# DaehwanKimLab/centrifuge

Measured on AMD Instinct MI355X. Metric: classified reads/sec (whole node) on 100bp synthetic reads vs p_compressed; HBM GB/s achieved, higher is better.
Workload: dtype u64

## Files before the change

### centrifuge_amd/csrc/cf_device.hip

```cpp
#include <hip/hip_runtime.h>
#include <sched.h>
#include <dlfcn.h>

#include <algorithm>
#include <cmath>
#include <chrono>
#include <cstdio>
#include <cstdlib>
#include <cstring>
#include <memory>
#include <mutex>
#include <stdexcept>
#include <string>
#include <vector>

#include "../../include/centrifuge_amd.h"
#include "cf_index.hpp"
#include "cf_kernels.hpp"
#include "cf_scan.hpp"
#include "cf_textio.hpp"
#include "cf_inflate.hpp"
#include "cf_restore.hpp"
#include "cf_plan.hpp"
#include "cf_knobs.hpp"
// ... 1285 lines not shown
    bt->maxLenHost = maxLen;
    const uint64_t nq = bt->nQueries;
    bt->bases.ensure(nWords + 16); bt->nmask.ensure(nWords + 16);
    bt->rlen.ensure(nReads + 16); bt->seeds.ensure(nReads + 1); bt->woff.ensure(nReads + 1);
    bt->pass.ensure(nReads + 1); bt->hitCap.ensure(nReads + 16);
    bt->slotOf.ensure(nReads + 1); bt->hitBase.ensure(nReads + 1); bt->items.ensure(nReads + 1);
    bt->nhml.ensure(2 * nReads + 1);
    bt->maxScore.ensure(nq + 1); bt->qflag.ensure(nq + 1); bt->qhead.ensure(nq + 1); bt->qRows.ensure(nq + 16); bt->qBase.ensure(nq + 1);
    bt->qplan.ensure((nq + 1) * kInlinePlan); bt->o1tax.ensure((nq + 1) * kFieldRows); bt->o1a.ensure((nq + 1) * kFieldRows); bt->o1b.ensure((nq + 1) * kFieldRows);
    bt->slowPost.ensure(nq + 1); bt->slowScore.ensure(nq + 1);
    if (envInt("CF_EARLY_SCORE", 0)) bt->postDeferred.ensure(nq + 16);
    bt->out.ensure(nq * (uint64_t)cl->d.k + 1); bt->nOut.ensure(nq + 16); bt->score2.ensure(nq + 1); bt->rowFirst.ensure(nq + 1);
    bt->cursor.ensure(4); bt->ops.ensure(1); bt->st.ensure(1);
    bt->tileA.ensure(scan_tiles_for(std::max(nReads, nq)) + 1); bt->tileC.ensure(scan_tiles_for(std::max(nReads, nq)) + 1);
    bt->recWords = searchVersion() != 2 ? 0u : maxLen <= 128 ? 4u : maxLen <= 192 ? 6u : maxLen <= 256 ? 8u : 0u;
    if ((uint64_t)(0.15 * maxLen) + maxLen / (uint64_t)ftc + 3 >= 255) bt->recWords = 0;
    bt->selfRecords = bt->recWords && cl->ix->d.planes && nWords < 0xffffffffull && envInt("CF_SELF_RECORDS", 1);
    if (bt->selfRecords) bt->itemMeta.ensure(8 * nReads + 8);
    bt->revDelta = bt->selfRecords && 2 * nWords + 64 < 0xffffffffull && envInt("CF_REV_WORDS", 1) ? (uint32_t)nWords + 16u : 0u;
    if (bt->revDelta) bt->bases.ensure(2 * (nWords + 16));
    else if (bt->recWords) bt->recs.ensure(2 * nReads * (uint64_t)rec_bytes((int)bt->recWords) + 64);
    uint64_t hitsWant = 2 * ((nBases ? nBases : 32 * nWords) / ftc + 2 * nReads);
    hitsWant += hitsWant / 50 + 4096;
    if (bt->hitsCapLimit) hitsWant = std::min(hitsWant, bt->hitsCapLimit);
    if (bt->hits.n < hitsWant) bt->hits.ensure(hitsWant);
    if (bt->recWords && bt->hits.n > 0xffffffffull) throw ArgError("batch too large: its hit lists need 32-bit offsets, split it");
    uint64_t rowsWant = std::max<uint64_t>(4 * nq, 1u << 16);
    if (bt->plannedPerQuery > 0) rowsWant = std::max<uint64_t>(rowsWant, (uint64_t)((double)nq * bt->plannedPerQuery * 1.15));
    if (const int per = envInt("CF_ROWS_PER_QUERY", 0)) rowsWant = std::max<uint64_t>((uint64_t)per * nq, 1024);
    if (bt->rowsCapLimit) rowsWant = bt->rowsCapLimit;
    if (bt->rowVal.n < rowsWant || bt->rowsCapLimit) { bt->rowVal.ensure(rowsWant); bt->rowRef.ensure(rowsWant); bt->hm.ensure(rowsWant); bt->tc.ensure(rowsWant); }
    bt->outCompact.ensure(nq * (uint64_t)cl->d.k + 1);
    bt->hSt.ensure(1); bt->hOps.ensure(1);
    bt->hNOut.ensure(nq + 1); bt->hScore2.ensure(nq + 1); bt->hMaxScore.ensure(nq + 1);
    if (bt->resultFormat == CF_RESULTS_NARROW) { bt->qinfo.ensure(nq + 16); bt->hQInfo.ensure(nq + 16); }
    bt->rowsSpec = bt->rowsPerQuery > 0 ? (uint64_t)((double)nq * bt->rowsPerQuery * 1.04) + 4096 : nq + nq / 4 + 1024;
    bt->rowsSpec = std::min<uint64_t>(bt->rowsSpec, nq * (uint64_t)cl->d.k);
    bt->hRows.ensure(std::max<uint64_t>(bt->rowsSpec, nq + nq / 4 + 1024));
    if (g_dryBytes) return;
    if (!bt->evInit) { for (auto &e : bt->ev) HIP_OK(hipEventCreate(&e)); HIP_OK(hipEventCreate(&bt->evLate)); HIP_OK(hipEventCreate(&bt->evPostFast)); HIP_OK(hipEventCreate(&bt->evPost)); bt->evInit = true; }
    if (!bt->tail && (envInt("CF_TAIL_STREAM", 0) || envInt("CF_EARLY_SCORE", 0))) HIP_OK(hipStreamCreateWithFlags(&bt->tail, hipStreamNonBlocking));
}

static void bindBatch(cf_batch *bt) {
    cf_classifier *cl = bt->cl;
    DPlan &pl = bt->pl;
    pl.nmask = bt->nmask.p; pl.rlen = bt->rlen.p; pl.woff = bt->woff.p; pl.nReads = (uint32_t)bt->nReads; pl.ftabChars = cl->ix->h.g.ftabChars;
    pl.maxLenAllowed = bt->maxLenHost;
    pl.nWords = bt->nWords;
    pl.pass = bt->pass.p; pl.hitCap = bt->hitCap.p; pl.slotOf = bt->slotOf.p;
    pl.hitBase = bt->hitBase.p; pl.items = bt->items.p; pl.st = bt->st.p;
    pl.itemMeta = bt->selfRecords ? bt->itemMeta.p : nullptr;
    pl.bases = bt->bases.p; pl.revDelta = bt->revDelta;
    pl.hitsCap = bt->hitsCapLimit ? std::min<uint64_t>(bt->hitsCapLimit, bt->hits.n) : bt->hits.n;
    DBatch &d = bt->d;
    d.bases = bt->bases.p; d.nmask = bt->nmask.p; d.rlen = bt->rlen.p; d.woff = bt->woff.p; d.seeds = bt->seeds.p;
    d.pass = bt->pass.p; d.items = bt->items.p; d.slotOf = bt->slotOf.p; d.hitBase = bt->hitBase.p; d.hitCap = bt->hitCap.p;
    d.lazyHits = (uint32_t)(envInt("CF_LAZY_HITS", 1) != 0) | (cl->ix->d.posFrag ? 4u : 0u);
    d.directRefs = (uint32_t)(cl->ix->dense.p && cl->ix->d.walkRate == 0 && envInt("CF_SCORE_FAST", 1) != 0 && envInt("CF_DIRECT_REFS", 1) != 0);
    d.hits = bt->hits.p; d.nhml = bt->nhml.p; d.qflag = bt->qflag.p; d.qhead = bt->qhead.p; d.qplan = bt->qplan.p; d.qplanStride = bt->qplan.n / kInlinePlan; d.qRows = bt->qRows.p; d.qBase = bt->qBase.p;
    d.rowVal = bt->rowVal.p; d.rowRef = bt->rowRef.p; d.hm = bt->hm.p; d.tc = bt->tc.p;
    d.out = bt->out.p; d.nOut = bt->nOut.p; d.score2 = bt->score2.p;
    d.counts = cl->counts.p; d.nTaxa = (uint32_t)cl->ix->h.taxa.size();
    d.nReads = (uint32_t)bt->nReads; d.nQueries = (uint32_t)bt->nQueries; d.paired = bt->paired;
    d.cursor = bt->cursor.p; d.st = bt->st.p; d.ops = bt->ops.p;
    d.slowPost = bt->slowPost.p; d.slowScore = bt->slowScore.p; d.postDeferred = envInt("CF_EARLY_SCORE", 0) ? bt->postDeferred.p : nullptr;
    d.o1tax = bt->o1tax.p; d.o1a = bt->o1a.p; d.o1b = bt->o1b.p; d.oStride = bt->o1tax.n / kFieldRows;
    d.hitsCap = pl.hitsCap;
    d.rowsCap = bt->rowsCapLimit ? std::min<uint64_t>(bt->rowsCapLimit, bt->rowVal.n) : bt->rowVal.n;
    d.recs = bt->recWords && !bt->selfRecords ? bt->recs.p : nullptr; d.recWords = bt->recWords;
    d.itemMeta = bt->selfRecords ? bt->itemMeta.p : nullptr;
}

static void enqueuePlan(cf_batch *bt, hipStream_t st) {
    const uint64_t nReads = bt->nReads;
    const DPlan &pl = bt->pl;
    HIP_OK(hipStreamWaitEvent(st, bt->ev[8], 0));
    if (bt->densePending) {
        const uint32_t L = bt->densePending - 1;
        const DUnpack u{bt->dense.p, bt->bases.p, bt->rlen.p, (uint32_t)nReads, L, bt->revDelta ? bt->bases.p + bt->revDelta : nullptr};
        bt->revMade = bt->revDelta != 0;
        const uint64_t threads = nReads * std::max<uint64_t>(((uint64_t)L + 31) >> 5, 1);
        hipLaunchKernelGGL(k_dense_unpack, dim3((unsigned)((threads + 255) / 256)), dim3(256), 0, st, u);
        bt->densePending = 0;
    }
    HIP_OK(hipEventRecord(bt->ev[5], st));
    HIP_OK(hipMemsetAsync(bt->st.p, 0, sizeof(BatchStatus), st));
    const dim3 gp((unsigned)((nReads + 1 + 255) / 256)), bl(256);
    if (bt->fromBytes && nReads) hipLaunchKernelGGL(k_rlen, gp, bl, 0, st, bt->off8.p, bt->rlen.p, (uint32_t)nReads);
    scan_enqueue<SCAN_WORDS>(bt->rlen.p, nReads, bt->woff.p, nullptr, bt->tileA.p, bt->tileC.p, st);
    if (bt->fromBytes && nReads) {
        DConvert c{bt->seq.p, bt->off8.p, bt->woff.p, bt->bases.p, bt->nmask.p, (uint32_t)nReads};
        hipLaunchKernelGGL(k_convert, dim3((unsigned)((nReads + 255) / 256)), dim3(256), 0, st, c);
    }
    if (bt->fromText && nReads) {
        const DTextPack c{bt->text.p, bt->txSeqOff.p, bt->rlen.p, bt->woff.p, bt->bases.p, bt->nmask.p, (uint32_t)nReads};
        hipLaunchKernelGGL(k_text_pack, dim3((unsigned)((nReads + 255) / 256)), dim3(256), 0, st, c);
    }
    hipLaunchKernelGGL(k_plan, gp, bl, 0, st, pl);
    scan_enqueue<SCAN_HITS>(bt->hitCap.p, nReads, bt->hitBase.p, bt->slotOf.p, bt->tileA.p, bt->tileC.p, st);
    hipLaunchKernelGGL(k_plan_fill, gp, bl, 0, st, pl);
    if (pl.revDelta && nReads && !bt->revMade) {
        const uint64_t threads = nReads * (uint64_t)bt->recWords;
        hipLaunchKernelGGL(k_rev_words, dim3((unsigned)((threads + 255) / 256)), bl, 0, st, pl, bt->recWords);
    }
    if (bt->nQueries) hipLaunchKernelGGL(k_plan_maxscore, dim3((unsigned)((bt->nQueries + 255) / 256)), bl, 0, st, bt->rlen.p, bt->pass.p,
// ... 1252 lines not shown
```

### centrifuge_amd/csrc/cf_kernels.hpp

```cpp
#pragma once
#include "cf_platform.hpp"

namespace cfamd {

constexpr uint32_t kNone32 = 0xffffffffu;
constexpr uint64_t kNone64 = ~0ull;
constexpr uint32_t kSideChars = 384;
constexpr int kSearchChunk = CF_WAVE;

struct RefInfo { uint64_t tax; uint32_t tidx, pid; };
static_assert(sizeof(RefInfo) == 16, "RefInfo layout");
struct DIndex {
    const uint8_t *sides;
    const uint64_t *ftab, *eftab;
    uint64_t fchr0, fchr1, fchr2, fchr3;
    uint64_t len, zOff, zSide;
    uint32_t zIn;
    int32_t ftabChars, offRate, offw;
    const void *offs;
    const uint8_t *planes;
    const uint8_t *planes2;
    const uint64_t *wide;
    int32_t wideChars;
    const uint64_t *text;
// ... 466 lines not shown
    uint64_t *rev;
};
CF_DEV void dense_unpack_body(const DUnpack &u, uint64_t t) {
    const uint32_t W = (u.readLen + 31) >> 5, bpr = (u.readLen + 3) >> 2;
    if (W == 0) { if (t < u.nReads) u.rlen[t] = 0; return; }
    const uint64_t r = t / W;
    const uint32_t k = (uint32_t)(t - r * W);
    if (r >= u.nReads) return;
    uint64_t w = load8_any(u.dense, r * bpr + 8ull * k);
    const uint32_t have = u.readLen - 32 * k;
    if (have < 32) w &= (1ull << (2 * have)) - 1;
    u.bases[r * W + k] = w;
    if (k == 0) u.rlen[r] = u.readLen;
    if (u.rev) {
        const uint32_t L = u.readLen;
        const int32_t s0 = (int32_t)(L - 1 - 32u * k) - 31;
        uint64_t x;
        if (s0 >= 0) {
            const uint64_t at = r * bpr + ((uint32_t)s0 >> 2);
            const uint32_t sh = 2u * ((uint32_t)s0 & 3u);
            x = load8_any(u.dense, at) >> sh;
            if (sh) x |= (load8_any(u.dense, at + 8) & 0xffull) << (64 - sh);
        } else x = load8_any(u.dense, r * bpr) << (2 * (uint32_t)(-s0));
        uint64_t rv = pair_reverse(x);
        if (have < 32) rv &= (1ull << (2 * have)) - 1;
        u.rev[r * W + k] = rv;
    }
}

CF_DEV void rlen_body(const uint64_t *off, uint32_t *rlen, uint32_t nReads, uint32_t r) {
    if (r >= nReads) return;
    const uint64_t l = off[r + 1] - off[r];
    rlen[r] = l > 0xffffffffull ? 0xffffffffu : (uint32_t)l;
}

struct DPlan {
    const uint32_t *nmask;
    const uint32_t *rlen;
    const uint64_t *woff;
    uint32_t nReads;
    int32_t ftabChars;
    uint32_t maxLenAllowed;
    uint64_t nWords;
    uint8_t *pass;
    uint32_t *hitCap;
    uint32_t *slotOf;
    uint64_t *hitBase;
    uint32_t *items;
    uint32_t *itemMeta;
    uint64_t *bases;
    uint32_t revDelta;
    BatchStatus *st;
    uint64_t hitsCap;
};

CF_DEV void plan_body(const DPlan &p, uint32_t r) {
    if (r < p.nReads) {
        const uint64_t L = p.rlen[r], wo = p.woff[r];
        uint32_t nN = 0;
        const bool inside = wo + ((L + 31) >> 5) <= p.nWords;
        if (!inside) cf_atomic_or(&p.st->flags, kStWordsOverflow);
        for (uint64_t k = 0; inside && 32 * k < L; k++) {
            uint32_t m = p.nmask[wo + k];
            if (L - 32 * k < 32) m &= (1u << (L - 32 * k)) - 1u;
            nN += (uint32_t)cf_popc32(m);
        }
        const uint64_t maxns = (uint64_t)(0.0 + (double)0.15f * (double)L);
        bool ok = inside && L >= 2 && nN <= maxns;
        if (ok && L > p.maxLenAllowed) { cf_atomic_or(&p.st->flags, kStLenOverflow); ok = false; }
        const uint32_t cap = ok ? (uint32_t)(nN + (L - nN) / (uint64_t)p.ftabChars + 2) : 0u;
        p.pass[r] = ok ? 1 : 0;
        p.hitCap[r] = cap;
    }
}

CF_DEV uint64_t rev_word(const uint64_t *rw, uint32_t L, uint32_t k) {
    const uint32_t have = L - 32u * k;
    const int32_t s0 = (int32_t)(L - 1 - 32u * k) - 31;
    uint64_t x;
    if (s0 >= 0) {
        const uint32_t wi = (uint32_t)s0 >> 5, sh = (uint32_t)s0 & 31;
        x = rw[wi] >> (2 * sh);
        if (sh) x |= rw[wi + 1] << (64 - 2 * sh);
    } else x = rw[0] << (2 * (uint32_t)(-s0));
    uint64_t w = pair_reverse(x);
    if (have < 32) w &= (1ull << (2 * have)) - 1;
    return w;
}

constexpr uint32_t kItemHasN = 0x80000000u;
constexpr uint32_t kItemPre = 0x40000000u;
CF_DEV void plan_fill_body(const DPlan &p, uint32_t r) {
    if (r > p.nReads) return;
    if (r == p.nReads) {
        const uint64_t need = p.hitBase[r];
        p.st->hitsNeed = need;
        if (need > p.hitsCap) { cf_atomic_or(&p.st->flags, kStHitsOverflow); p.st->nItems = 0; }
        else p.st->nItems = 2u * p.slotOf[r];
        return;
    }
    const uint32_t slot = p.slotOf[r];
    if (p.pass[r]) {
        p.items[slot] = r;
        if (p.itemMeta) {
            const uint32_t wo = (uint32_t)p.woff[r], L = p.rlen[r], hb = (uint32_t)p.hitBase[r];
            uint32_t any = 0;
            for (uint32_t k = 0; 32 * k < L; k++) {
                uint32_t mk = p.nmask[p.woff[r] + k];
                if (L - 32 * k < 32) mk &= (1u << (L - 32 * k)) - 1u;
                any |= mk;
            }
            const bool pre = p.revDelta && !any;
            const uint32_t Lf = L | (any ? kItemHasN : 0u) | (pre ? kItemPre : 0u);
            uint32_t *m = p.itemMeta + 8 * (size_t)slot;
            m[0] = pre ? wo + p.revDelta : wo; m[1] = Lf; m[2] = hb; m[3] = r;
            m[4] = wo; m[5] = Lf; m[6] = hb + p.hitCap[r]; m[7] = r;
        }
    } else p.slotOf[r] = kNone32;
}

CF_DEV void rev_words_body(const DPlan &p, uint32_t wordsPerRead, uint64_t t) {
    const uint64_t r = t / wordsPerRead;
    const uint32_t k = (uint32_t)(t - r * wordsPerRead);
    if (r >= p.nReads || !p.revDelta || !p.pass[r]) return;
    const uint32_t L = p.rlen[r];
    if (32u * k >= L) return;
    const uint64_t wo = p.woff[r];
    p.bases[wo + p.revDelta + k] = rev_word(p.bases + wo, L, k);
}

constexpr uint32_t kMaxScoreNever = 0xffffffffu;
CF_DEV void plan_maxscore_body(const uint32_t *rlen, const uint8_t *pass, uint32_t nQueries, int paired, uint32_t *maxScore, uint32_t q) {
    if (q >= nQueries) return;
    const uint32_t r0 = paired ? 2 * q : q;
    const uint64_t L0 = rlen[r0];
    const uint64_t s0 = L0 > 15 ? (L0 - 15) * (L0 - 15) : 0u;
    const bool p0 = pass[r0] != 0;
    uint64_t v = p0 ? s0 : 0u;
    if (paired) {
        const uint64_t L1 = rlen[r0 + 1];
        const uint64_t s1 = L1 > 15 ? (L1 - 15) * (L1 - 15) : 0u;
        const bool p1 = pass[r0 + 1] != 0;
        v = (p0 && p1) ? s0 + s1 : p0 ? s0 : p1 ? s1 : 0u;
    }
    maxScore[q] = v >= 0xffffffffull ? kMaxScoreNever : (uint32_t)v;
}

struct DCompact {
    const OutRow *out;
    const uint64_t *o1tax, *o1a, *o1b;
    uint64_t oStride;
    const uint32_t *nOut;
    const uint64_t *rowFirst;
    uint32_t k, nQueries;
    OutRow *dst;
    BatchStatus *st;
    NarrowRow *dstNarrow;
    uint8_t *qinfo;
    const uint8_t *pass;
    int32_t paired;
};
CF_DEV OutRow row_of_one(uint64_t tax, uint64_t a, uint64_t bb) {
    OutRow o; o.taxID = tax; o.uniqueID = (uint32_t)a; o.score = (uint32_t)(a >> 32); o.hitLen = (uint32_t)bb; o.tidx = (uint32_t)(bb >> 32);
    return o;
}
CF_DEV void compact_body(const DCompact &c, uint32_t q) {
    if (q == c.nQueries && c.st) c.st->rowsOut = c.rowFirst[q];
    if (q >= c.nQueries) return;
    const uint32_t n = c.nOut[q] < c.k ? c.nOut[q] : c.k;
// ... 411 lines not shown
                rank_any<1>(ix, c0, t1, b1, t2, b2, two);
                if (b2 > t2) m4 |= 1u << c0;
            }
            if (!m4) masked = false;
            mask |= m4 << (4 * c1);
        }
    }
    table[t] = wide_entry(top, bot - top, j - ftc, cap, masked, mask);
}

enum : int { S_IDLE = 0, S_REC = 1, S_CALL = 2, S_FTAB = 3, S_EXT = 4, S_EXTB = 5, S_FTABW = 6, S_POS = 7, S_TXT = 8, S_ISA = 9, S_REC2 = 10 };

constexpr uint32_t kLazyHits = 2;
constexpr uint32_t lazy_hits(int G, int W) { return G == 1 && W >= 6 ? 1u : kLazyHits; }
constexpr uint32_t kVerifyMinLeft = 12;

template <int G, int W, bool COUNT, bool BLOCKS = false, int LZN = 0, bool MULTI = false>
CF_DEV void search2_body(const DIndex &ix, const DParams &pr, const DBatch &b, uint8_t *ldsBlock) {
    static_assert(!BLOCKS || G == 1, "the planes are read one chain per lane");
    constexpr int PER = 8 / G;
    constexpr int RB = rec_bytes(W);
    constexpr int RCH = RB / (16 * G);
    constexpr int NV = BLOCKS ? (RCH > 2 ? RCH : 2) : PER;
    static_assert(RCH >= 1 && RCH <= NV, "record does not fit the load slot");
    constexpr uint32_t kRawPieces = W / 2 + (W + 3) / 4;
    static_assert(G != 1 || (int)kRawPieces <= NV, "packed read does not fit the load slot");
    struct Slot { u64x2 v[NV]; };
    const int sub = Grp<G>::sub();
    const uint32_t lane = cf_lane();
    const uint32_t leaderLane = lane & ~(uint32_t)(G - 1);
    constexpr int RBL = rec_lds_stride(W);
    uint8_t *lrec = ldsBlock + (size_t)(cf_local_thread() / G) * RBL;
    constexpr uint32_t LZ = LZN ? (uint32_t)LZN : lazy_hits(G, W);
    uint64_t *lhit = reinterpret_cast<uint64_t *>(ldsBlock + (size_t)(cf_block_threads() / G) * RBL +
                                                  (BLOCKS ? (size_t)0 : (size_t)cf_block_threads() * 4 * RankTab<G>::WORDS)) +
                     (size_t)(cf_local_thread() / G) * 2 * LZ;
    uint32_t *scr = BLOCKS ? nullptr : reinterpret_cast<uint32_t *>(ldsBlock + (size_t)(cf_block_threads() / G) * RBL) + (size_t)cf_local_thread() * RankTab<G>::WORDS;
    const uint64_t *lw = reinterpret_cast<const uint64_t *>(lrec);
    const uint32_t *lm = reinterpret_cast<const uint32_t *>(lrec + 8 * W);
    uint32_t *lmeta = reinterpret_cast<uint32_t *>(lrec + RB - 16);
    const uint32_t ftc = (uint32_t)ix.ftabChars;
    int mode = S_IDLE;
    uint32_t cur = 0, dep = 0;
    uint32_t nhmx = 0;
    uint64_t top = 0, bot = 0;
    uint64_t aux = 0;
    uint32_t vf = 0;
    uint32_t endDep = 0;
    uint32_t mv = 0;
    uint32_t lz = 0;
    uint32_t wnext = 0, wend = 0;
    bool exhausted = false;
    constexpr bool SELF = G == 1;
    u64x2 cmeta{0, 0};
    uint32_t cbase = 0, pend = 0;
    unsigned long long cFtab = 0, cPair = 0, cPair2 = 0, cSingle = 0, cFtabW = 0, cVerify = 0, cText = 0, cPos = 0;
    const int32_t posRate = ix.posRate;
    const int32_t isaRate = MULTI ? posRate : ix.isaRate;
    const uint32_t nItems = b.st->nItems;
    const uint32_t wideChars = (uint32_t)ix.wideChars;

    for (;;) {
        uint32_t item = 0;
        const bool selfRec = SELF && b.itemMeta != nullptr;
        auto takeMeta = [&](bool mine, uint32_t it) {
            const int src = (int)((mine ? it - cbase : lane) & (uint32_t)(CF_WAVE - 1));
            const uint32_t m0 = cf_shfl((uint32_t)cmeta.x, src), m1 = cf_shfl((uint32_t)(cmeta.x >> 32), src), m2 = cf_shfl((uint32_t)cmeta.y, src);
            if (mine) {
                aux = (uint64_t)m0 | ((uint64_t)(m1 & (kItemHasN | kItemPre)) << 32);
                lmeta[0] = m1 & ~(kItemHasN | kItemPre); lmeta[1] = m2; lmeta[2] = it;
                cf_compiler_fence();
                mode = S_REC2;
            }
        };
        if (selfRec && cf_ballot(mode == S_REC)) takeMeta(mode == S_REC, pend);
        const uint64_t idleMask = cf_ballot(mode == S_IDLE && sub == 0);
        if (idleMask) {
            bool fresh = false;
            if (wnext >= wend && !exhausted) {
                uint32_t base = 0;
                if (lane == 0) base = (uint32_t)cf_atomic_add(&b.cursor[0], (unsigned long long)kSearchChunk);
                base = cf_first_lane_u32(base);
                if (base >= nItems) { exhausted = true; wnext = wend = 0; }
                else {
                    wnext = base; wend = base + kSearchChunk < nItems ? base + kSearchChunk : nItems;
                    if (selfRec) {
                        cbase = base; fresh = true;
                        cmeta = base + lane < nItems ? cf_load16(reinterpret_cast<const uint8_t *>(b.itemMeta + 4 * (size_t)(base + lane))) : u64x2{0, 0};
                    }
                }
            }
            const uint32_t avail = wend - wnext;
            const uint32_t nIdle = (uint32_t)cf_popc64(idleMask);
            bool took = false;
            if (mode == S_IDLE) {
                const uint32_t rnk = (uint32_t)cf_popc64(idleMask & ((1ull << leaderLane) - 1));
                if (rnk < avail) { item = wnext + rnk; mode = S_REC; pend = item; took = true; }
            }
            wnext += nIdle < avail ? nIdle : avail;
            if (selfRec && !fresh && cf_ballot(took)) takeMeta(took, item);
        }
        if (cf_ballot(mode != S_IDLE) == 0) {
            if (exhausted) break;
            continue;
        }
        const bool anyN = cf_ballot((mode != S_IDLE && (lz & 2u) != 0) || (mode == S_REC2 && (aux >> 63) != 0) || (mode == S_REC && !selfRec)) != 0;
        auto iter = [&](auto lmx) __attribute__((always_inline)) {
        Slot sa;
        sa.v[0] = u64x2{0, 0};
        uint64_t sS = 0;
        uint32_t oT = 0, oB = 0;
        bool same = true, stepN = false;
        int c = 0;
        const uint8_t *ldp = nullptr;
        uint32_t nch = 0, strd = 16;
        if (posRate >= 0 && mode == S_EXT && !(vf & 25u) && bot - top == 1 && (vf >> 8) >= ix.verifyMinRun &&
            (top & ((1ull << posRate) - 1)) == 0 && lmeta[0] - dep >= kVerifyMinLeft) {
            mode = S_POS;
            if (COUNT) cVerify++;
        } else if (MULTI && G == 1 && posRate == 0 && ix.multiRows && mode == S_EXT && !(vf & 25u) && bot - top >= 2 && bot - top <= ix.multiRows &&
                   (vf >> 8) >= ix.multiMinRun && lmeta[0] - dep >= kVerifyMinLeft) {
            mv = 0x80000000u | ((uint32_t)(bot - top) << 20);
            endDep = dep;
            mode = S_POS;
            if (COUNT) cVerify++;
        }
        if (mode == S_POS) {
            const uint64_t row = top + ((MULTI && (mv >> 31)) ? (mv & 15u) : 0u);
            if (COUNT && (MULTI && (mv >> 31)) && (mv & 15u)) cText++;
            ldp = reinterpret_cast<const uint8_t *>(ix.saPos + 2 * ((row >> posRate) / 3)); nch = 1;
        } else if (mode == S_ISA) {
            ldp = reinterpret_cast<const uint8_t *>(ix.isa + 2 * ((aux >> isaRate) / 3)); nch = 1;
        } else if (mode == S_TXT) {
            if constexpr (G == 1) {
                const uint64_t b0 = aux >= 64 ? ((aux - 1) >> 5) - 1 : 0;
                ldp = reinterpret_cast<const uint8_t *>(ix.text) + 8 * b0; nch = 1;
            } else {
                const uint64_t b0 = aux >= 64 ? (aux - 64) >> 5 : 0;
                ldp = reinterpret_cast<const uint8_t *>(ix.text) + 8 * b0 + (size_t)sub * (32 / G); nch = 2 / G;
            }
            if (COUNT) cText++;
        } else if (mode == S_REC) {
            if (G == 1 && b.itemMeta) nch = 0;
            else { ldp = b.recs + (uint64_t)item * RB + (size_t)sub * (RB / G); nch = RCH; }
        } else if (G == 1 && mode == S_REC2) {
            ldp = reinterpret_cast<const uint8_t *>(b.bases + (uint32_t)aux); nch = (aux >> 63) ? kRawPieces : W / 2;
        } else if (mode == S_FTAB) {
            ldp = reinterpret_cast<const uint8_t *>(ix.ftab + aux); nch = 1;
        } else if (mode == S_FTABW) {
            ldp = reinterpret_cast<const uint8_t *>(ix.wide + aux); nch = 1;
        } else if (mode == S_EXT || mode == S_EXTB) {
            c = (int)((lw[dep >> 5] >> (2 * (dep & 31))) & 3);
            stepN = mode == S_EXT && ((lmx[dep >> 5] >> (dep & 31)) & 1u) != 0;
            if (!stepN) {
                if constexpr (BLOCKS) {
                    const uint64_t row = mode == S_EXT ? top : bot;
                    sS = row >> 6;
                    if (mode == S_EXT) {
                        oT = (uint32_t)row & 63u;
                        const uint64_t spread = bot - top;
                        same = (uint64_t)oT + spread <= 64;
                        oB = same ? oT + (uint32_t)spread : 0u;
                        const uint32_t d1 = dep + 1;
                        const bool pair = ix.planes2 && !(vf & 8u) && d1 < lmeta[0] && ((lmx[d1 >> 5] >> (d1 & 31)) & 1u) == 0 &&
                                          !((vf & 16u) && d1 >= endDep);
                        vf = pair ? (vf | 4u) : (vf & ~4u);
                    } else oB = (uint32_t)row & 63u;
                    if (vf & 4u) {
                        const uint32_t d1 = dep + 1;
                        const int c0 = (int)((lw[d1 >> 5] >> (2 * (d1 & 31))) & 3);
                        ldp = ix.planes2 + sS * 256 + 16 * (4 * c + c0); nch = 1;
                    } else { ldp = ix.planes + sS * 64 + 16 * c; nch = 1; }
                } else {
                    if (mode == S_EXT) {
                        sS = side_of(ix, top);
                        oT = (uint32_t)(top - sS * kSideChars);
                        const uint64_t spread = bot - top;
                        same = (uint64_t)oT + spread <= kSideChars;
                        oB = same ? oT + (uint32_t)spread : 0u;
                    } else {
                        sS = side_of(ix, bot);
                        oB = (uint32_t)(bot - sS * kSideChars);
                    }
                    ldp = ix.sides + sS * 128 + 16 * sub; nch = PER; strd = 16 * G;
                }
            }
        }
        if (nch) sa.v[0] = cf_load16(ldp);
        if (nch > 1) {
#pragma unroll
            for (int i = 1; i < NV; i++) {
                if ((uint32_t)i >= nch) continue;
                if (G == 1 && mode == S_REC2 && i >= W / 2) sa.v[i] = cf_load16(reinterpret_cast<const uint8_t *>(b.nmask + (uint32_t)aux) + 16 * (i - W / 2));
                else sa.v[i] = cf_load16(ldp + (size_t)i * strd);
            }
        }
        cf_wait_vmem();
        const u64x2 ft = sa.v[0];
// ... 108 lines not shown
                for (int k = 0; k < W; k++) {
                    const uint64_t v = (k & 1) ? sa.v[k / 2].y : sa.v[k / 2].x;
                    uint64_t w = 0;
                    if (32u * (uint32_t)k < L) {
                        const uint32_t have = L - 32u * (uint32_t)k;
                        w = fwd ? v : ~v;
                        if (have < 32) w &= (1ull << (2 * have)) - 1;
                    }
                    rw[k] = w; rm[k] = 0u;
                }
            } else {
#pragma unroll
            for (int i = 0; i < W / 2; i++) { rw[2 * i] = sa.v[i].x; rw[2 * i + 1] = sa.v[i].y; }
#pragma unroll
            for (int i = 0; i < (W + 3) / 4; i++) {
                const bool hasN = (aux >> 63) != 0;
                const uint64_t a = hasN ? sa.v[W / 2 + i].x : 0ull, bq = hasN ? sa.v[W / 2 + i].y : 0ull;
                if (4 * i + 0 < W) rm[4 * i + 0] = (uint32_t)a;
                if (4 * i + 1 < W) rm[4 * i + 1] = (uint32_t)(a >> 32);
                if (4 * i + 2 < W) rm[4 * i + 2] = (uint32_t)bq;
                if (4 * i + 3 < W) rm[4 * i + 3] = (uint32_t)(bq >> 32);
            }
            cf_compiler_fence();
            uint64_t fw_[W]; uint32_t fm_[W];
#pragma unroll
            for (int k = 0; k < W; k++) {
                uint64_t w = 0; uint32_t m = 0;
                if (32u * (uint32_t)k < L) {
                    const uint32_t have = L - 32u * (uint32_t)k;
                    if (fwd) {
                        const int32_t s0 = (int32_t)(L - 1 - 32u * (uint32_t)k) - 31;
                        uint64_t x; uint32_t mm;
                        if (s0 >= 0) {
                            const uint32_t wi = (uint32_t)s0 >> 5, sh = (uint32_t)s0 & 31;
                            x = lw[wi] >> (2 * sh); mm = lmx[wi] >> sh;
                            if (sh) { x |= lw[wi + 1] << (64 - 2 * sh); mm |= lmx[wi + 1] << (32 - sh); }
                        } else {
                            const uint32_t neg = (uint32_t)(-s0);
                            x = lw[0] << (2 * neg); mm = lmx[0] << neg;
                        }
                        w = pair_reverse(x); m = cf_brev32(mm);
                    } else { w = ~lw[k]; m = lmx[k]; }
                    if (have < 32) { w &= (1ull << (2 * have)) - 1; m &= (1u << have) - 1u; }
                    w &= ~spread_pairs(m);
                }
                fw_[k] = w; fm_[k] = m;
            }
            cf_compiler_fence();
#pragma unroll
            for (int k = 0; k < W; k++) { rw[k] = fw_[k]; rm[k] = fm_[k]; }
            }
            cf_compiler_fence();
            cur = 0; nhmx = 0; lz = (b.lazyHits & 5u) | ((aux >> 63) ? 2u : 0u);
            mode = S_CALL;
        } else if (mode == S_REC) {
            uint64_t *dst = reinterpret_cast<uint64_t *>(lrec + (size_t)sub * (RB / G));
#pragma unroll
            for (int i = 0; i < RCH; i++) { dst[2 * i] = sa.v[i].x; dst[2 * i + 1] = sa.v[i].y; }
            cf_compiler_fence();
            static_assert(12 * W <= RB - 16, "words and masks must not reach into the meta chunk");
            if (sub == G - 1) lmeta[2] = item;
            cf_compiler_fence();
            cur = 0; nhmx = 0; lz = (b.lazyHits & 5u) | 2u;
            mode = S_CALL;
        } else if (mode == S_FTABW) {
            const uint64_t size = wide_size(ft.x);
            if (size == kWideSizeMax) {
                aux &= (1ull << (2 * ftc)) - 1;
                mode = S_FTAB;
                if (COUNT) cFtab++;
            } else if (size == 0) {
                push = true; pLen = ftc; cur += ftc;
            } else {
                const uint32_t D = ftc + (uint32_t)((ft.x >> 40) & 15u);
                top = ft.x & ((1ull << 40) - 1); bot = top + size;
                dep = cur + D;
                const uint32_t L = lmeta[0];
                bool ends = D < wideChars || dep >= L;
                constexpr uint32_t kUnknownMore = 0xffu;
                uint32_t more = kUnknownMore;
                if (!ends && wide_masked(ft.x) && ((lmx[dep >> 5] >> (dep & 31)) & 1u) == 0) {
                    const uint32_t code = (uint32_t)(ft.x >> 44) & 15u, d1 = dep + 1;
                    if (kWideCtxRows > 0 && code <= kWideCtxRows) {
                        const uint32_t nb = wide_ctx_bases(code);
                        const uint32_t k = dep >> 5, sh = dep & 31;
                        uint32_t q = (uint32_t)(lw[k] >> (2 * sh)), nm = lmx[k] >> sh;
                        if (sh > 24) { q |= (uint32_t)(lw[k + 1] << (64 - 2 * sh)); nm |= lmx[k + 1] << (32 - sh); }
                        uint32_t lim = L - dep < nb ? L - dep : nb;
                        nm &= (1u << nb) - 1u;
                        if (nm) { const uint32_t fn = (uint32_t)cf_ctz32(nm); if (fn < lim) lim = fn; }
                        const uint32_t pay = (uint32_t)(ft.x >> 48);
                        uint32_t mmax = 0, nmax = 0, rmax = 0;
#pragma unroll
                        for (uint32_t r = 0; r < (kWideCtxRows ? (uint32_t)kWideCtxRows : 1u); r++) {
                            if (r >= code) continue;
                            uint32_t x = ((pay >> (2 * nb * r)) ^ q) & ((1u << (2 * nb)) - 1u);
                            x = (x | (x >> 1)) & 0x5555u;
                            uint32_t mr = x ? (uint32_t)cf_ctz32(x) >> 1 : nb;
                            if (mr > lim) mr = lim;
                            if (mr > mmax) { mmax = mr; nmax = 1; rmax = r; } else if (mr == mmax) nmax++;
                        }
                        if (mmax == nb && nmax == 1) { top += rmax; bot = top + 1; }
                        if (mmax < nb) more = mmax;
                    } else {
                        const int c1 = (int)((lw[dep >> 5] >> (2 * (dep & 31))) & 3);
                        const uint32_t m4 = (uint32_t)(ft.x >> (48 + 4 * c1)) & 15u;
                        if (!m4) more = 0;
                        else if (d1 >= L || ((lmx[d1 >> 5] >> (d1 & 31)) & 1u) != 0 || !((m4 >> ((lw[d1 >> 5] >> (2 * (d1 & 31))) & 3)) & 1u)) more = 1;
                    }
                    if (more == 0) ends = true;
                    else if (more != kUnknownMore) {
                        if ((lz & 1u) && (nhmx & 0xffu) >= LZ && D + more < pr.m) {
                            push = true; pTop = top; pBot = bot; pLen = D + more; cur = dep + more;
                        } else {
                            vf |= 16u; endDep = dep + more;
                            if (BLOCKS && ix.planes2 && more == 1) vf |= 8u;
                            mode = S_EXT;
                        }
                    } else mode = S_EXT;
                } else if (!ends) mode = S_EXT;
                if (ends) { push = true; pTop = top; pBot = bot; pLen = D; cur = dep; }
            }
        } else if (mode == S_FTAB) {
            top = ft.x <= ix.len ? ft.x : ix.eftab[(ft.x ^ kNone64) * 2 + 1];
            bot = ft.y <= ix.len ? ft.y : ix.eftab[(ft.y ^ kNone64) * 2];
            dep = cur + ftc;
            if (bot <= top) { push = true; pLen = ftc; cur = dep; }
            else if (dep >= lmeta[0]) { push = true; pTop = top; pBot = bot; pLen = dep - (nhmx >> 20); cur = dep; }
            else mode = S_EXT;
        } else if (mode == S_EXT || mode == S_EXTB) {
            bool stop = stepN;
            if (!stepN) {
                if (COUNT && mode == S_EXT) {
                    if (bot - top > 1) cPair++; else cSingle++;
                    if (!same) cPair2++;
                }
                if constexpr (!BLOCKS) rank_tab_build<G>(reinterpret_cast<const Side<G> &>(sa), pat32(c), scr);
                uint64_t t, bb;
                if constexpr (BLOCKS) {
                    t = sa.v[0].y + popc_below(sa.v[0].x, oT);
                    bb = sa.v[0].y + popc_below(sa.v[0].x, oB);
                } else if constexpr (G == 2) {
                    const uint64_t occ = sub == (c >> 1) ? ((c & 1) ? sa.v[8 / G - 1].y : sa.v[8 / G - 1].x) : 0ull;
                    uint64_t pT = rank_tab_count<G>(scr, oT) + occ;
                    uint64_t pB = rank_tab_count<G>(scr, oB) + occ;
                    pT += swap1_64(pT);
                    pB += swap1_64(pB);
                    t = pT; bb = pB;
                } else {
                    uint32_t acc = rank_tab_count<G>(scr, oT) | (rank_tab_count<G>(scr, oB) << 16);
                    acc = Grp<G>::sum(acc);
                    const uint64_t occ = side_occ<G>(reinterpret_cast<const Side<G> &>(sa), c);
                    t = occ + (acc & 0xffffu);
                    bb = occ + (acc >> 16);
                }
                if constexpr (!BLOCKS) {
                    if (c == 0 && sS == ix.zSide) {
                        if (ix.zIn < oT) t--;
                        if (ix.zIn < oB) bb--;
                    }
                    const uint64_t f = fchr_of(ix, c);
                    t += f; bb += f;
                }
                if (mode == S_EXT && !same) {
                    aux = t;
                    mode = S_EXTB;
                } else {
                    if (mode == S_EXTB) { t = aux; mode = S_EXT; }
                    const bool pair = BLOCKS && (vf & 4u) != 0;
                    if (bb <= t) {
                        if (pair) vf = (vf & ~4u) | 8u;
                        else stop = true;
                    } else {
                        vf = bb - t == bot - top ? vf + (pair ? 0x200u : 0x100u) : (vf & 0xffu);
                        top = t; bot = bb; dep += pair ? 2u : 1u; stop = dep >= lmeta[0] || (vf & 8u) != 0 || ((vf & 16u) && dep == endDep);
                        vf &= ~4u;
                    }
                }
            }
            if (stop) { push = true; pTop = top; pBot = bot; pLen = dep - (nhmx >> 20); cur = dep; }
        }
        auto emitHit = [&](uint64_t w0, uint64_t w1, uint32_t hlen) -> bool {
            const uint32_t j = nhmx & 0xffu;
            HitP *dst = b.hits + ((uint64_t)lmeta[1] + j);
            if (!(lz & 1u)) { if (sub == 0) cf_store16_stream(dst, w0, w1); return false; }
            if (hlen >= pr.m) {
                if (j > LZ) return true;
                if (sub == 0) {
#pragma unroll
                    for (uint32_t t = 0; t < LZ; t++) if (t < j) cf_store16_stream(dst - j + t, lhit[2 * t], lhit[2 * t + 1]);
                    cf_store16_stream(dst, w0, w1);
                }
                lz &= ~1u;
                return false;
            }
            if (j < LZ && sub == 0) { lhit[2 * j] = w0; lhit[2 * j + 1] = w1; }
            return false;
        };
        if (push) {
            const uint32_t L = lmeta[0];
            const bool dummy = pTop == kNone64;
            const bool posf = !dummy && (pTop & kRowIsPos) != 0;
            if (emitHit((dummy ? kHit40 : (pTop & kHit40)) | ((uint64_t)pLen << 40), (dummy ? 0ull : posf ? (1ull | kHitPosForm) : pBot - pTop) | ((uint64_t)(nhmx >> 20) << 40), pLen)) {
                cur = 0; nhmx = 0; lz &= ~1u; mode = S_CALL;
            } else {
                { const uint32_t mx = (nhmx >> 8) & 0xfffu; nhmx = (nhmx & 0xfff000ffu) + 1u + ((pLen > mx ? pLen : mx) << 8); }
                bool done = cur >= L;
                if (!done) {
                    if (pLen > pr.inc) cur += 1;
                    done = cur + pr.m >= L;
                }
                if (done) { if (sub == 0) b.nhml[lmeta[2]] = nhml_make(nhmx & 0xffu, ((nhmx >> 8) & 0xfffu) >= pr.m); mode = S_IDLE; }
                else mode = S_CALL;
            }
        }
        if (mode == S_CALL) {
            const uint32_t L = lmeta[0];
            nhmx = (nhmx & 0xfffffu) | (cur << 20);
            vf = 0; mv = 0;
            uint32_t len = 0, newCur = 0;
            const int how = ps_begin2(lw, lmx, L, cur, ftc, wideChars, aux, len, newCur);
            if (how == 2) { mode = S_FTABW; if (COUNT) cFtabW++; }
            else if (how == 1) { mode = S_FTAB; if (COUNT) cFtab++; }
            else {
                if (emitHit(kHit40 | ((uint64_t)len << 40), (uint64_t)(nhmx >> 20) << 40, len)) {
                    cur = 0; nhmx = 0; lz &= ~1u;
                } else {
                    { const uint32_t mx = (nhmx >> 8) & 0xfffu; nhmx = (nhmx & 0xfff000ffu) + 1u + ((len > mx ? len : mx) << 8); }
                    cur = newCur;
                    bool done = cur >= L;
                    if (!done) {
                        if (len > pr.inc) cur += 1;
                        done = cur + pr.m >= L;
// ... 1284 lines not shown
```

Before: 1.429 billion.

## Precompute first wide-ftab index in plan and prefetch it with read bases

The plan-fill kernel now computes the first wide-ftab lookup key for each strand of N-free reads and stores it in the item metadata, replacing the redundant read index. The search kernel shuffles this key, issues the wide-ftab load together with the read-bases load in the record-loading state, and then jumps directly into the wide-ftab handling. The S_FTABW handler is moved out of the else-if chain so it can run in the same iteration. This removes one dependent memory round trip per query start, at the cost of extra metadata logic and a wider load slot.

```diff
diff --git a/centrifuge_amd/csrc/cf_device.hip b/centrifuge_amd/csrc/cf_device.hip
--- a/centrifuge_amd/csrc/cf_device.hip
+++ b/centrifuge_amd/csrc/cf_device.hip
@@ -1361,6 +1361,8 @@
     pl.hitBase = bt->hitBase.p; pl.items = bt->items.p; pl.st = bt->st.p;
     pl.itemMeta = bt->selfRecords ? bt->itemMeta.p : nullptr;
     pl.bases = bt->bases.p; pl.revDelta = bt->revDelta;
+    static const bool firstLookup = envInt("CF_FIRST_LOOKUP", 1) != 0;
+    pl.wideChars = bt->selfRecords && firstLookup && cl->ix->d.wide && cl->ix->d.wideChars > 0 && !cl->ix->d.multiRows ? (uint32_t)cl->ix->d.wideChars : 0u;
     pl.hitsCap = bt->hitsCapLimit ? std::min<uint64_t>(bt->hitsCapLimit, bt->hits.n) : bt->hits.n;
     DBatch &d = bt->d;
     d.bases = bt->bases.p; d.nmask = bt->nmask.p; d.rlen = bt->rlen.p; d.woff = bt->woff.p; d.seeds = bt->seeds.p;
diff --git a/centrifuge_amd/csrc/cf_kernels.hpp b/centrifuge_amd/csrc/cf_kernels.hpp
--- a/centrifuge_amd/csrc/cf_kernels.hpp
+++ b/centrifuge_amd/csrc/cf_kernels.hpp
@@ -542,6 +542,7 @@
     uint32_t revDelta;
     BatchStatus *st;
     uint64_t hitsCap;
+    uint32_t wideChars;
 };
 
 CF_DEV void plan_body(const DPlan &p, uint32_t r) {
@@ -580,6 +581,10 @@
 
 constexpr uint32_t kItemHasN = 0x80000000u;
 constexpr uint32_t kItemPre = 0x40000000u;
+constexpr uint32_t kItemFirst = 0x20000000u;
+#ifdef CF_HOST_EMU
+inline unsigned long long g_emuFirstTaken = 0, g_emuFirstBad = 0;
+#endif
 CF_DEV void plan_fill_body(const DPlan &p, uint32_t r) {
     if (r > p.nReads) return;
     if (r == p.nReads) {
@@ -601,10 +606,17 @@
                 any |= mk;
             }
             const bool pre = p.revDelta && !any;
-            const uint32_t Lf = L | (any ? kItemHasN : 0u) | (pre ? kItemPre : 0u);
+            const bool first = p.wideChars && p.wideChars <= 16 && L >= p.wideChars && !any;
+            const uint32_t Lf = L | (any ? kItemHasN : 0u) | (pre ? kItemPre : 0u) | (first ? kItemFirst : 0u);
+            uint32_t fiF = r, fiR = r;
+            if (first) {
+                const uint32_t km = (uint32_t)((1ull << (2 * p.wideChars)) - 1);
+                fiF = (uint32_t)rev_word(p.bases + p.woff[r], L, 0) & km;
+                fiR = (uint32_t)~p.bases[p.woff[r]] & km;
+            }
             uint32_t *m = p.itemMeta + 8 * (size_t)slot;
-            m[0] = pre ? wo + p.revDelta : wo; m[1] = Lf; m[2] = hb; m[3] = r;
-            m[4] = wo; m[5] = Lf; m[6] = hb + p.hitCap[r]; m[7] = r;
+            m[0] = pre ? wo + p.revDelta : wo; m[1] = Lf; m[2] = hb; m[3] = fiF;
+            m[4] = wo; m[5] = Lf; m[6] = hb + p.hitCap[r]; m[7] = fiR;
         }
     } else p.slotOf[r] = kNone32;
 }
@@ -1122,6 +1134,7 @@
     uint32_t wnext = 0, wend = 0;
     bool exhausted = false;
     constexpr bool SELF = G == 1;
+    constexpr bool FIRST = G == 1 && !MULTI;
     u64x2 cmeta{0, 0};
     uint32_t cbase = 0, pend = 0;
     unsigned long long cFtab = 0, cPair = 0, cPair2 = 0, cSingle = 0, cFtabW = 0, cVerify = 0, cText = 0, cPos = 0;
@@ -1136,9 +1149,12 @@
         auto takeMeta = [&](bool mine, uint32_t it) {
             const int src = (int)((mine ? it - cbase : lane) & (uint32_t)(CF_WAVE - 1));
             const uint32_t m0 = cf_shfl((uint32_t)cmeta.x, src), m1 = cf_shfl((uint32_t)(cmeta.x >> 32), src), m2 = cf_shfl((uint32_t)cmeta.y, src);
+            uint32_t m3 = 0;
+            if constexpr (FIRST) m3 = cf_shfl((uint32_t)(cmeta.y >> 32), src);
             if (mine) {
-                aux = (uint64_t)m0 | ((uint64_t)(m1 & (kItemHasN | kItemPre)) << 32);
-                lmeta[0] = m1 & ~(kItemHasN | kItemPre); lmeta[1] = m2; lmeta[2] = it;
+                aux = (uint64_t)m0 | ((uint64_t)(m1 & (kItemHasN | kItemPre | kItemFirst)) << 32);
+                if constexpr (FIRST) top = m3;
+                lmeta[0] = m1 & ~(kItemHasN | kItemPre | kItemFirst); lmeta[1] = m2; lmeta[2] = it;
                 cf_compiler_fence();
                 mode = S_REC2;
             }
@@ -1214,6 +1230,7 @@
             if (G == 1 && b.itemMeta) nch = 0;
             else { ldp = b.recs + (uint64_t)item * RB + (size_t)sub * (RB / G); nch = RCH; }
         } else if (G == 1 && mode == S_REC2) {
+            if (FIRST && ((aux >> 61) & 1u)) sa.v[W / 2] = cf_load16(reinterpret_cast<const uint8_t *>(ix.wide + (uint32_t)top));
             ldp = reinterpret_cast<const uint8_t *>(b.bases + (uint32_t)aux); nch = (aux >> 63) ? kRawPieces : W / 2;
         } else if (mode == S_FTAB) {
             ldp = reinterpret_cast<const uint8_t *>(ix.ftab + aux); nch = 1;
@@ -1428,7 +1445,15 @@
             }
             cf_compiler_fence();
             cur = 0; nhmx = 0; lz = (b.lazyHits & 5u) | ((aux >> 63) ? 2u : 0u);
-            mode = S_CALL;
+            if (FIRST && ((aux >> 61) & 1u)) {
+                aux = (uint32_t)top; sa.v[0].x = sa.v[W / 2].x;
+                vf = 0; mv = 0;
+                mode = S_FTABW;
+                if (COUNT) cFtabW++;
+#ifdef CF_HOST_EMU
+                { uint64_t fi = 0; uint32_t l0 = 0, n0 = 0; g_emuFirstTaken++; if (ps_begin2(lw, lmx, L, 0u, ftc, wideChars, fi, l0, n0) != 2 || fi != aux) g_emuFirstBad++; }
+#endif
+            } else mode = S_CALL;
         } else if (mode == S_REC) {
             uint64_t *dst = reinterpret_cast<uint64_t *>(lrec + (size_t)sub * (RB / G));
 #pragma unroll
@@ -1439,64 +1464,6 @@
             cf_compiler_fence();
             cur = 0; nhmx = 0; lz = (b.lazyHits & 5u) | 2u;
             mode = S_CALL;
-        } else if (mode == S_FTABW) {
-            const uint64_t size = wide_size(ft.x);
-            if (size == kWideSizeMax) {
-                aux &= (1ull << (2 * ftc)) - 1;
-                mode = S_FTAB;
-                if (COUNT) cFtab++;
-            } else if (size == 0) {
-                push = true; pLen = ftc; cur += ftc;
-            } else {
-                const uint32_t D = ftc + (uint32_t)((ft.x >> 40) & 15u);
-                top = ft.x & ((1ull << 40) - 1); bot = top + size;
-                dep = cur + D;
-                const uint32_t L = lmeta[0];
-                bool ends = D < wideChars || dep >= L;
-                constexpr uint32_t kUnknownMore = 0xffu;
-                uint32_t more = kUnknownMore;
-                if (!ends && wide_masked(ft.x) && ((lmx[dep >> 5] >> (dep & 31)) & 1u) == 0) {
-                    const uint32_t code = (uint32_t)(ft.x >> 44) & 15u, d1 = dep + 1;
-                    if (kWideCtxRows > 0 && code <= kWideCtxRows) {
-                        const uint32_t nb = wide_ctx_bases(code);
-                        const uint32_t k = dep >> 5, sh = dep & 31;
-                        uint32_t q = (uint32_t)(lw[k] >> (2 * sh)), nm = lmx[k] >> sh;
-                        if (sh > 24) { q |= (uint32_t)(lw[k + 1] << (64 - 2 * sh)); nm |= lmx[k + 1] << (32 - sh); }
-                        uint32_t lim = L - dep < nb ? L - dep : nb;
-                        nm &= (1u << nb) - 1u;
-                        if (nm) { const uint32_t fn = (uint32_t)cf_ctz32(nm); if (fn < lim) lim = fn; }
-                        const uint32_t pay = (uint32_t)(ft.x >> 48);
-                        uint32_t mmax = 0, nmax = 0, rmax = 0;
-#pragma unroll
-                        for (uint32_t r = 0; r < (kWideCtxRows ? (uint32_t)kWideCtxRows : 1u); r++) {
-                            if (r >= code) continue;
-                            uint32_t x = ((pay >> (2 * nb * r)) ^ q) & ((1u << (2 * nb)) - 1u);
-                            x = (x | (x >> 1)) & 0x5555u;
-                            uint32_t mr = x ? (uint32_t)cf_ctz32(x) >> 1 : nb;
-                            if (mr > lim) mr = lim;
-                            if (mr > mmax) { mmax = mr; nmax = 1; rmax = r; } else if (mr == mmax) nmax++;
-                        }
-                        if (mmax == nb && nmax == 1) { top += rmax; bot = top + 1; }
-                        if (mmax < nb) more = mmax;
-                    } else {
-                        const int c1 = (int)((lw[dep >> 5] >> (2 * (dep & 31))) & 3);
-                        const uint32_t m4 = (uint32_t)(ft.x >> (48 + 4 * c1)) & 15u;
-                        if (!m4) more = 0;
-                        else if (d1 >= L || ((lmx[d1 >> 5] >> (d1 & 31)) & 1u) != 0 || !((m4 >> ((lw[d1 >> 5] >> (2 * (d1 & 31))) & 3)) & 1u)) more = 1;
-                    }
-                    if (more == 0) ends = true;
-                    else if (more != kUnknownMore) {
-                        if ((lz & 1u) && (nhmx & 0xffu) >= LZ && D + more < pr.m) {
-                            push = true; pTop = top; pBot = bot; pLen = D + more; cur = dep + more;
-                        } else {
-                            vf |= 16u; endDep = dep + more;
-                            if (BLOCKS && ix.planes2 && more == 1) vf |= 8u;
-                            mode = S_EXT;
-                        }
-                    } else mode = S_EXT;
-                } else if (!ends) mode = S_EXT;
-                if (ends) { push = true; pTop = top; pBot = bot; pLen = D; cur = dep; }
-            }
         } else if (mode == S_FTAB) {
             top = ft.x <= ix.len ? ft.x : ix.eftab[(ft.x ^ kNone64) * 2 + 1];
             bot = ft.y <= ix.len ? ft.y : ix.eftab[(ft.y ^ kNone64) * 2];
@@ -1555,6 +1522,66 @@
                 }
             }
             if (stop) { push = true; pTop = top; pBot = bot; pLen = dep - (nhmx >> 20); cur = dep; }
+        }
+        if (mode == S_FTABW) {
+            const uint64_t fw0 = sa.v[0].x;
+            const uint64_t size = wide_size(fw0);
+            if (size == kWideSizeMax) {
+                aux &= (1ull << (2 * ftc)) - 1;
+                mode = S_FTAB;
+                if (COUNT) cFtab++;
+            } else if (size == 0) {
+                push = true; pLen = ftc; cur += ftc;
+            } else {
+                const uint32_t D = ftc + (uint32_t)((fw0 >> 40) & 15u);
+                top = fw0 & ((1ull << 40) - 1); bot = top + size;
+                dep = cur + D;
+                const uint32_t L = lmeta[0];
+                bool ends = D < wideChars || dep >= L;
+                constexpr uint32_t kUnknownMore = 0xffu;
+                uint32_t more = kUnknownMore;
+                if (!ends && wide_masked(fw0) && ((lmx[dep >> 5] >> (dep & 31)) & 1u) == 0) {
+                    const uint32_t code = (uint32_t)(fw0 >> 44) & 15u, d1 = dep + 1;
+                    if (kWideCtxRows > 0 && code <= kWideCtxRows) {
+                        const uint32_t nb = wide_ctx_bases(code);
+                        const uint32_t k = dep >> 5, sh = dep & 31;
+                        uint32_t q = (uint32_t)(lw[k] >> (2 * sh)), nm = lmx[k] >> sh;
+                        if (sh > 24) { q |= (uint32_t)(lw[k + 1] << (64 - 2 * sh)); nm |= lmx[k + 1] << (32 - sh); }
+                        uint32_t lim = L - dep < nb ? L - dep : nb;
+                        nm &= (1u << nb) - 1u;
+                        if (nm) { const uint32_t fn = (uint32_t)cf_ctz32(nm); if (fn < lim) lim = fn; }
+                        const uint32_t pay = (uint32_t)(fw0 >> 48);
+                        uint32_t mmax = 0, nmax = 0, rmax = 0;
+#pragma unroll
+                        for (uint32_t r = 0; r < (kWideCtxRows ? (uint32_t)kWideCtxRows : 1u); r++) {
+                            if (r >= code) continue;
+                            uint32_t x = ((pay >> (2 * nb * r)) ^ q) & ((1u << (2 * nb)) - 1u);
+                            x = (x | (x >> 1)) & 0x5555u;
+                            uint32_t mr = x ? (uint32_t)cf_ctz32(x) >> 1 : nb;
+                            if (mr > lim) mr = lim;
+                            if (mr > mmax) { mmax = mr; nmax = 1; rmax = r; } else if (mr == mmax) nmax++;
+                        }
+                        if (mmax == nb && nmax == 1) { top += rmax; bot = top + 1; }
+                        if (mmax < nb) more = mmax;
+                    } else {
+                        const int c1 = (int)((lw[dep >> 5] >> (2 * (dep & 31))) & 3);
+                        const uint32_t m4 = (uint32_t)(fw0 >> (48 + 4 * c1)) & 15u;
+                        if (!m4) more = 0;
+                        else if (d1 >= L || ((lmx[d1 >> 5] >> (d1 & 31)) & 1u) != 0 || !((m4 >> ((lw[d1 >> 5] >> (2 * (d1 & 31))) & 3)) & 1u)) more = 1;
+                    }
+                    if (more == 0) ends = true;
+                    else if (more != kUnknownMore) {
+                        if ((lz & 1u) && (nhmx & 0xffu) >= LZ && D + more < pr.m) {
+                            push = true; pTop = top; pBot = bot; pLen = D + more; cur = dep + more;
+                        } else {
+                            vf |= 16u; endDep = dep + more;
+                            if (BLOCKS && ix.planes2 && more == 1) vf |= 8u;
+                            mode = S_EXT;
+                        }
+                    } else mode = S_EXT;
+                } else if (!ends) mode = S_EXT;
+                if (ends) { push = true; pTop = top; pBot = bot; pLen = D; cur = dep; }
+            }
         }
         auto emitHit = [&](uint64_t w0, uint64_t w1, uint32_t hlen) -> bool {
             const uint32_t j = nhmx & 0xffu;
```

Result: no change. 1.424 billion (-0.4%).
